# wtfashwin/fraud-detection

Measured on AMD Instinct MI355X. Metric: train_rows_per_sec (SMOTE k-NN + logistic fit, post-SMOTE rows/s, whole job); AUC; SHAP values/s, higher is better.
Workload: dtype bf16; 1 GPU; model=StandardScaler+SMOTE(k=5)+LogisticRegression(C=1,sgd), global_batch=8000000, seq_len=30, parallelism=dp1, rows_per_gpu=10000000, post_smote_rows_global=15972800, smote_scope=global

## Files before the change

fraud_detection_amd/csrc/kernels/knn.hip:

```cpp
#include <cmath>
#include <cstdlib>

#include "common.h"
#include "launchers.h"
#include "scaler_finalize.h"

namespace fdx {
namespace {

constexpr int kThreads = 256;
constexpr int kWaves = 4;
constexpr int kMaxK = 8;
constexpr float kNegBig = -3.0e38f;
constexpr int kQFlush = 4;
constexpr int kQCap = kQFlush - 1 + 16 + 1;

__device__ __forceinline__ bool better(float s, int i, float s2, int i2) {
  return s > s2 || (s == s2 && i < i2);
}

template <int K>
__device__ __forceinline__ void topk_insert(float (&bs)[K], int (&bi)[K], float s, int i) {
  if (!better(s, i, bs[K - 1], bi[K - 1])) return;
  bs[K - 1] = s;
  bi[K - 1] = i;
#pragma unroll
  for (int k = K - 1; k > 0; --k) {
    if (better(bs[k], bi[k], bs[k - 1], bi[k - 1])) {
      const float ts = bs[k]; bs[k] = bs[k - 1]; bs[k - 1] = ts;
      const int ti = bi[k]; bi[k] = bi[k - 1]; bi[k - 1] = ti;
    }
  }
}

__device__ __forceinline__ void split_row(const float (&x)[32], uint32_t (&h)[16], uint32_t (&l)[16]);
template <bool RAW>
__device__ __forceinline__ float4 prep_load(const float4* __restrict__ p, int k, const float* st, int d) {
#pragma clang fp contract(off)
  float4 v = p[k];
  if constexpr (RAW) {
    const int c = 4 * k;
    if (c < d) v.x = (v.x - st[c]) * st[32 + c];
    if (c + 1 < d) v.y = (v.y - st[c + 1]) * st[32 + c + 1];
    if (c + 2 < d) v.z = (v.z - st[c + 2]) * st[32 + c + 2];
    if (c + 3 < d) v.w = (v.w - st[c + 3]) * st[32 + c + 3];
  }
  return v;
}
template <bool RAW>
__device__ __forceinline__ void knn_prep_body(const float* __restrict__ X, int m, int m_pad, int role,
                                              float* __restrict__ out, float* __restrict__ outq,
                                              const double* __restrict__ aff, uint16_t* __restrict__ P,
                                              uint4* __restrict__ chl, uint4* __restrict__ qhl,
                                              float* __restrict__ tmax, const float* st, int d) {
#pragma clang fp contract(off)
  const int r = blockIdx.x * blockDim.x + threadIdx.x;
  if (chl != nullptr) {
    const bool ok = r < m_pad;
    float x[32];
    if (ok && r < m) {
      const float4* p = reinterpret_cast<const float4*>(X + (int64_t)r * kCols);
      float s = 0.0f;
#pragma unroll
      for (int k = 0; k < kCols / 4; ++k) {
        float4 v = prep_load<RAW>(p, k, st, d);
        if (k == kCols / 4 - 1) {
          s = fmaf(v.x, v.x, s); s = fmaf(v.y, v.y, s);
          v.z = 0.0f; v.w = 0.0f;
        } else {
          s = fmaf(v.x, v.x, s); s = fmaf(v.y, v.y, s); s = fmaf(v.z, v.z, s); s = fmaf(v.w, v.w, s);
        }
        x[4 * k] = v.x; x[4 * k + 1] = v.y; x[4 * k + 2] = v.z; x[4 * k + 3] = v.w;
      }
      x[30] = -0.5f * s;
    } else {
#pragma unroll
      for (int k = 0; k < 32; ++k) x[k] = 0.0f;
      x[30] = -3.0e38f;
    }
    uint32_t h[16], l[16];
    split_row(x, h, l);
    if (ok) {
      const int64_t tb = (int64_t)(r >> 5) * 256 + (r & 31);
#pragma unroll
      for (int v = 0; v < 8; ++v) {
        const int k = v & 3;
        const uint4 c = v < 4 ? make_uint4(h[4 * k], h[4 * k + 1], h[4 * k + 2], h[4 * k + 3])
                              : make_uint4(l[4 * k], l[4 * k + 1], l[4 * k + 2], l[4 * k + 3]);
        chl[tb + (v >> 1) * 64 + (v & 1) * 32] = c;
      }
    }
    float n2 = (ok && x[30] > -1.0e37f) ? -2.0f * x[30] : 0.0f;
#pragma unroll
    for (int o = 1; o < 32; o <<= 1) n2 = fmaxf(n2, __shfl_xor(n2, o, kWave));
    if (ok && (r & 31) == 0) tmax[r >> 5] = sqrtf(n2) * 1.0001f;
    x[30] = (ok && r < m) ? 1.0f : 0.0f;
    split_row(x, h, l);
    if (ok) {
#pragma unroll
      for (int k = 0; k < 4; ++k) {
        qhl[(int64_t)r * 8 + k] = make_uint4(h[4 * k], h[4 * k + 1], h[4 * k + 2], h[4 * k + 3]);
        qhl[(int64_t)r * 8 + 4 + k] = make_uint4(l[4 * k], l[4 * k + 1], l[4 * k + 2], l[4 * k + 3]);
      }
    }
  }
  if (r >= m_pad) return;
  float4* o = reinterpret_cast<float4*>(out + (int64_t)r * kCols);
  float4* oq = role == 2 ? reinterpret_cast<float4*>(outq + (int64_t)r * kCols) : nullptr;
  if (r >= m) {
#pragma unroll
    for (int k = 0; k < kCols / 4; ++k) {
      o[k] = make_float4(0.f, 0.f, 0.f, 0.f);
      if (oq) oq[k] = make_float4(0.f, 0.f, 0.f, 0.f);
    }
    if (role != 1) out[(int64_t)r * kCols + 30] = -3.0e38f;
    return;
  }
  const float4* p = reinterpret_cast<const float4*>(X + (int64_t)r * kCols);
  uint2* pp = P ? reinterpret_cast<uint2*>(P + (int64_t)r * kCols) : nullptr;
  float s = 0.0f;
#pragma unroll
  for (int k = 0; k < kCols / 4; ++k) {
    float4 v = prep_load<RAW>(p, k, st, d);
    if (pp) {
      float4 u = v;
      if constexpr (RAW) {
        const int c = 4 * k;
        u.x = u.x * st[64 + c] + st[96 + c];
        u.y = u.y * st[64 + c + 1] + st[96 + c + 1];
        if (c + 2 < kBiasCol) {
          u.z = u.z * st[64 + c + 2] + st[96 + c + 2];
          u.w = u.w * st[64 + c + 3] + st[96 + c + 3];
        }
      } else if (aff != nullptr) {
        const int c = 4 * k;
        u.x = u.x * (float)(1.0 / aff[32 + c]) + (float)aff[c];
        u.y = u.y * (float)(1.0 / aff[32 + c + 1]) + (float)aff[c + 1];
        if (c + 2 < kBiasCol) {
          u.z = u.z * (float)(1.0 / aff[32 + c + 2]) + (float)aff[c + 2];
          u.w = u.w * (float)(1.0 / aff[32 + c + 3]) + (float)aff[c + 3];
        }
      }
      pp[k] = make_uint2(pack_bf16x2(u.x, u.y), pack_bf16x2(u.z, u.w));
    }
    if (k == kCols / 4 - 1) {
      s = fmaf(v.x, v.x, s); s = fmaf(v.y, v.y, s);
      v.z = 0.0f; v.w = 0.0f;
    } else {
      s = fmaf(v.x, v.x, s); s = fmaf(v.y, v.y, s); s = fmaf(v.z, v.z, s); s = fmaf(v.w, v.w, s);
    }
    o[k] = v;
    if (oq) oq[k] = v;
  }
  out[(int64_t)r * kCols + 30] = role == 1 ? 1.0f : -0.5f * s;
  if (oq) outq[(int64_t)r * kCols + 30] = 1.0f;
}


__global__ void knn_prep_kernel(const float* __restrict__ X, int m, int m_pad, int role,
                                float* __restrict__ out, float* __restrict__ outq,
                                const double* __restrict__ aff, uint16_t* __restrict__ P,
                                uint4* __restrict__ chl = nullptr, uint4* __restrict__ qhl = nullptr,
                                float* __restrict__ tmax = nullptr) {
  knn_prep_body<false>(X, m, m_pad, role, out, outq, aff, P, chl, qhl, tmax, nullptr, 0);
}

__global__ __launch_bounds__(256) void knn_prep_raw_kernel(const float* __restrict__ X, int m, int m_pad,
                                                           float* __restrict__ out, float* __restrict__ outq,
                                                           uint16_t* __restrict__ P, uint4* __restrict__ chl,
                                                           uint4* __restrict__ qhl, float* __restrict__ tmax,
                                                           KnnRawStats st) {
  __shared__ float sst[4 * 32];
  if (threadIdx.x < 32) {
    const int c = threadIdx.x;
    float mu, inv;
    double ac, ai;
    if (st.nparts > 0) {
      const ScalerCol o = scaler_finalize_col(st.sums, st.n, st.pivot, st.d, st.colscale, st.nparts, c);
      mu = o.mean32; inv = o.inv32; ac = o.aff_c; ai = o.aff_inv;
      if (blockIdx.x == 0) {
        st.mean64[c] = o.mean; st.var64[c] = o.var; st.scale64[c] = o.scale;
        st.mean32[c] = mu; st.inv32[c] = inv;
        st.aff[c] = ac; st.aff[32 + c] = ai;
      }
    } else {
      mu = st.mean32[c]; inv = st.inv32[c]; ac = st.aff[c]; ai = st.aff[32 + c];
    }
    sst[c] = mu;
    sst[32 + c] = inv;
    sst[64 + c] = (float)(1.0 / ai);
    sst[96 + c] = (float)ac;
  }
  __syncthreads();
  knn_prep_body<true>(X, m, m_pad, 2, out, outq, nullptr, P, chl, qhl, tmax, sst, st.d);
}

template <int K, int QF = kQFlush>
__global__ __launch_bounds__(kWave) void knn_topk_kernel(const float* __restrict__ Q, int mq,
                                                         const float* __restrict__ C,
                                                         int mc_pad, int mc,
                                                         int64_t self_offset,
                                                         int* __restrict__ out_idx,
                                                         float* __restrict__ out_score) {
  const int lane = threadIdx.x;
  const int h = lane >> 5, j = lane & 31;
  const int q0 = blockIdx.x * 32;
  const int qg = q0 + j;
  const int64_t self_c = self_offset >= 0 ? self_offset + qg : -1;
  float bq[16];
  {
    const float4* p = reinterpret_cast<const float4*>(Q + (int64_t)qg * kCols + 16 * h);
#pragma unroll
    for (int k = 0; k < 4; ++k) {
      const float4 v = p[k];
      bq[4 * k] = v.x; bq[4 * k + 1] = v.y; bq[4 * k + 2] = v.z; bq[4 * k + 3] = v.w;
    }
  }
  float bs[K];
  int bi[K];
#pragma unroll
  for (int k = 0; k < K; ++k) { bs[k] = kNegBig; bi[k] = 0x7fffffff; }
  float thr = qg < mq ? kNegBig : __builtin_inff();

  constexpr int kCap = QF - 1 + 16 + 1;
  __shared__ int2 qent[kCap * kWave];
  int qn = 0;
  auto flush = [&]() {
    for (int e = 0; __any(e < qn); ++e) {
      if (e < qn) {
        const int2 v = qent[e * kWave + lane];
        const int ci = v.y;
        if (ci != self_c && ci < mc) topk_insert<K>(bs, bi, __int_as_float(v.x), ci);
      }
    }
    qn = 0;
    float ps[K];
#pragma unroll
    for (int k = 0; k < K; ++k) ps[k] = __shfl_xor(bs[k], 32, kWave);
    int ia = 0, ib = 0;
    float kth = kNegBig;
#pragma unroll
    for (int k = 0; k < K; ++k) {
      float a = kNegBig, b = kNegBig;
#pragma unroll
      for (int u = 0; u < K; ++u) { if (u == ia) a = bs[u]; if (u == ib) b = ps[u]; }
      const bool ta = a >= b;
      kth = ta ? a : b;
      ia += ta ? 1 : 0;
      ib += ta ? 0 : 1;
    }
    thr = qg < mq ? kth : __builtin_inff();
  };
  const int all_tiles = mc_pad / 32;
  const int t_lo = (int)(((int64_t)all_tiles * blockIdx.y) / gridDim.y);
  const int t_hi = (int)(((int64_t)all_tiles * (blockIdx.y + 1)) / gridDim.y);
  float4 cv[4];
  auto fetch = [&](int t, float4 (&a)[4]) {
    const float4* p = reinterpret_cast<const float4*>(C + (int64_t)(t * 32 + j) * kCols + 16 * h);
#pragma unroll
    for (int k = 0; k < 4; ++k) a[k] = p[k];
  };
  if (t_lo < t_hi) fetch(t_lo, cv);
  for (int t = t_lo; t < t_hi; ++t) {
    const int c0 = t * 32;
    float ac[16];
    f32x16_t acc = {};
#pragma unroll
    for (int k = 0; k < 4; ++k) {
      ac[4 * k] = cv[k].x; ac[4 * k + 1] = cv[k].y; ac[4 * k + 2] = cv[k].z; ac[4 * k + 3] = cv[k].w;
    }
    if (t + 1 < t_hi) fetch(t + 1, cv);
#pragma unroll
    for (int s = 0; s < 16; ++s) acc = __builtin_amdgcn_mfma_f32_32x32x2f32(ac[s], bq[s], acc, 0, 0, 0);
    float m4[4];
#pragma unroll
    for (int q = 0; q < 4; ++q) m4[q] = fmaxf(fmaxf(acc[4 * q], acc[4 * q + 1]), fmaxf(acc[4 * q + 2], acc[4 * q + 3]));
    const float mx = fmaxf(fmaxf(m4[0], m4[1]), fmaxf(m4[2], m4[3]));
    if (!__any(mx >= thr)) continue;
    const int cbase = c0 + 4 * h;
    int qe = qn * kWave + lane;
#pragma unroll
    for (int q = 0; q < 4; ++q) {
      if (!__any(m4[q] >= thr)) continue;
#pragma unroll
      for (int rr = 0; rr < 4; ++rr) {
        const int r = 4 * q + rr;
        const bool pass = acc[r] >= thr;
        if (__any(pass)) {
          if (pass) {
            qent[qe] = make_int2(__float_as_int(acc[r]), cbase + rr + 8 * q);
            qe += kWave;
          }
        }
      }
    }
    qn = (qe - lane) / kWave;
    if (__any(qn >= QF)) flush();
  }
  flush();
#pragma unroll
  for (int k = 0; k < K; ++k) {
    const float s2 = __shfl_xor(bs[k], 32, kWave);
    const int i2 = __shfl_xor(bi[k], 32, kWave);
    if (h == 0) topk_insert<K>(bs, bi, s2, i2);
  }
  if (h == 0 && qg < mq) {
    const int64_t o = ((int64_t)blockIdx.y * mq + qg) * K;
#pragma unroll
    for (int k = 0; k < K; ++k) {
      out_idx[o + k] = bi[k];
      if (out_score) out_score[o + k] = bs[k];
    }
  }
}

constexpr int kLW = 4;
constexpr int kCh = 2;
constexpr int kLdC = kCols + 4;

template <int K>
__global__ __launch_bounds__(kLW * kWave) void knn_topk_lds_kernel(const float* __restrict__ Q, int mq,
                                                                   const float* __restrict__ C, int mc_pad, int mc,
                                                                   int64_t self_offset, int* __restrict__ out_idx,
                                                                   float* __restrict__ out_score) {
  const int lane = lane_id(), wv = wave_id();
  const int h = lane >> 5, j = lane & 31;
  const int qg = (blockIdx.x * kLW + wv) * 32 + j;
  const int64_t self_c = self_offset >= 0 ? self_offset + qg : -1;
  __shared__ __attribute__((aligned(16))) float cbuf[2][kCh * 32 * kLdC];
  __shared__ int2 qall[kLW][kQCap * kWave];
  int2* qent = qall[wv];
  float bq[16];
  {
    const float4* p = reinterpret_cast<const float4*>(Q + (int64_t)qg * kCols + 16 * h);
#pragma unroll
    for (int k = 0; k < 4; ++k) {
      const float4 v = p[k];
      bq[4 * k] = v.x; bq[4 * k + 1] = v.y; bq[4 * k + 2] = v.z; bq[4 * k + 3] = v.w;
    }
  }
  float bs[K];
  int bi[K];
#pragma unroll
  for (int k = 0; k < K; ++k) { bs[k] = kNegBig; bi[k] = 0x7fffffff; }
  float thr = qg < mq ? kNegBig : __builtin_inff();
  int qn = 0;
  auto flush = [&]() {
    for (int e = 0; __any(e < qn); ++e) {
      if (e < qn) {
        const int2 v = qent[e * kWave + lane];
        const int ci = v.y;
        if (ci != self_c && ci < mc) topk_insert<K>(bs, bi, __int_as_float(v.x), ci);
      }
    }
    qn = 0;
    float ps[K];
#pragma unroll
    for (int k = 0; k < K; ++k) ps[k] = __shfl_xor(bs[k], 32, kWave);
    int ia = 0, ib = 0;
    float kth = kNegBig;
#pragma unroll
    for (int k = 0; k < K; ++k) {
      float a = kNegBig, b = kNegBig;
#pragma unroll
      for (int u = 0; u < K; ++u) { if (u == ia) a = bs[u]; if (u == ib) b = ps[u]; }
      const bool ta = a >= b;
      kth = ta ? a : b;
      ia += ta ? 1 : 0;
      ib += ta ? 0 : 1;
    }
    thr = qg < mq ? kth : __builtin_inff();
  };
  const int all_tiles = mc_pad / 32;
  const int t_lo = (int)(((int64_t)all_tiles * blockIdx.y) / gridDim.y);
  const int t_hi = (int)(((int64_t)all_tiles * (blockIdx.y + 1)) / gridDim.y);
  constexpr int kVec = kCh * 32 * 8 / (kLW * kWave);
  float4 st[kVec];
  auto load = [&](int c) {
    const int64_t r0 = (int64_t)(t_lo + kCh * c) * 32;
    const int64_t rmax = (int64_t)t_hi * 32;
#pragma unroll
    for (int i = 0; i < kVec; ++i) {
      const int e = threadIdx.x + i * kLW * kWave;
      const int64_t r = r0 + (e >> 3);
      st[i] = r < rmax ? reinterpret_cast<const float4*>(C + r * kCols)[e & 7] : make_float4(0.f, 0.f, 0.f, 0.f);
    }
  };
  auto store = [&](int b) {
#pragma unroll
    for (int i = 0; i < kVec; ++i) {
      const int e = threadIdx.x + i * kLW * kWave;
      *reinterpret_cast<float4*>(&cbuf[b][(e >> 3) * kLdC + 4 * (e & 7)]) = st[i];
    }
  };
  const int nch = (t_hi - t_lo + kCh - 1) / kCh;
  if (nch > 0) {
    load(0);
    store(0);
  }
  __syncthreads();
  for (int c = 0; c < nch; ++c) {
    if (c + 1 < nch) load(c + 1);
    const float* cb = cbuf[c & 1];
    const int ntile = min(kCh, t_hi - (t_lo + kCh * c));
    for (int tt = 0; tt < ntile; ++tt) {
      const int c0 = (t_lo + kCh * c + tt) * 32;
      const float* crow = cb + (tt * 32 + j) * kLdC + 16 * h;
      float ac[16];
#pragma unroll
      for (int k = 0; k < 4; ++k) {
        const float4 v = *reinterpret_cast<const float4*>(crow + 4 * k);
        ac[4 * k] = v.x; ac[4 * k + 1] = v.y; ac[4 * k + 2] = v.z; ac[4 * k + 3] = v.w;
      }
      f32x16_t acc = {};
#pragma unroll
      for (int s = 0; s < 16; ++s) acc = __builtin_amdgcn_mfma_f32_32x32x2f32(ac[s], bq[s], acc, 0, 0, 0);
      float mx = acc[0];
#pragma unroll
      for (int r = 1; r < 16; ++r) mx = fmaxf(mx, acc[r]);
      if (!__any(mx >= thr)) continue;
      const int cbase = c0 + 4 * h;
      int qe = qn * kWave + lane;
#pragma unroll
      for (int r = 0; r < 16; ++r) {
        const bool pass = acc[r] >= thr;
        if (__any(pass)) {
          if (pass) {
            qent[qe] = make_int2(__float_as_int(acc[r]), cbase + (r & 3) + 8 * (r >> 2));
            qe += kWave;
          }
        }
      }
      qn = (qe - lane) / kWave;
      if (__any(qn >= kQFlush)) flush();
    }
    if (c + 1 < nch) store((c + 1) & 1);
    __syncthreads();
  }
  flush();
#pragma unroll
  for (int k = 0; k < K; ++k) {
    const float s2 = __shfl_xor(bs[k], 32, kWave);
    const int i2 = __shfl_xor(bi[k], 32, kWave);
    if (h == 0) topk_insert<K>(bs, bi, s2, i2);
  }
  if (h == 0 && qg < mq) {
    const int64_t o = ((int64_t)blockIdx.y * mq + qg) * K;
#pragma unroll
    for (int k = 0; k < K; ++k) {
      out_idx[o + k] = bi[k];
      if (out_score) out_score[o + k] = bs[k];
    }
  }
}


__device__ __forceinline__ void split_row(const float (&x)[32], uint32_t (&h)[16], uint32_t (&l)[16]) {
#pragma unroll
  for (int k = 0; k < 16; ++k) {
    const float a = x[2 * k], b = x[2 * k + 1];
    const uint32_t ph = pack_bf16x2(a, b);
    h[k] = ph;
    l[k] = pack_bf16x2(a - bf16lo(ph), b - bf16hi(ph));
  }
}

__global__ __launch_bounds__(256) void knn_split_kernel(const float* __restrict__ Xp, int m_pad, int role,
                                                        uint4* __restrict__ hl, float* __restrict__ tmax) {
  const int r = blockIdx.x * 256 + threadIdx.x;
  const bool ok = r < m_pad;
  float x[32];
  const float4* p = reinterpret_cast<const float4*>(Xp + (int64_t)(ok ? r : 0) * kCols);
#pragma unroll
  for (int k = 0; k < 8; ++k) {
    const float4 v = p[k];
    x[4 * k] = v.x; x[4 * k + 1] = v.y; x[4 * k + 2] = v.z; x[4 * k + 3] = v.w;
  }
  uint32_t h[16], l[16];
  split_row(x, h, l);
  if (ok && role == 2) {
    const int64_t tb = (int64_t)(r >> 5) * 256 + (r & 31);
#pragma unroll
    for (int v = 0; v < 8; ++v) {
      const int k = v & 3;
      const uint4 c = v < 4 ? make_uint4(h[4 * k], h[4 * k + 1], h[4 * k + 2], h[4 * k + 3])
                            : make_uint4(l[4 * k], l[4 * k + 1], l[4 * k + 2], l[4 * k + 3]);
      hl[tb + (v >> 1) * 64 + (v & 1) * 32] = c;
    }
  } else if (ok) {
#pragma unroll
    for (int k = 0; k < 4; ++k) {
      hl[(int64_t)r * 8 + k] = make_uint4(h[4 * k], h[4 * k + 1], h[4 * k + 2], h[4 * k + 3]);
      hl[(int64_t)r * 8 + 4 + k] = make_uint4(l[4 * k], l[4 * k + 1], l[4 * k + 2], l[4 * k + 3]);
    }
  }
  if (role == 0 || role == 2) {
    float n2 = (ok && x[30] > -1.0e37f) ? -2.0f * x[30] : 0.0f;
// ... 568 lines not shown
  const int t_hi = (int)(((int64_t)all_tiles * (blockIdx.y + 1)) / gridDim.y);
  auto fetch = [&](int t, uint4 (&a)[4], float& tmv) {
    const uint4* p = Chl + (int64_t)t * 256 + lane;
    a[0] = p[0]; a[1] = p[64]; a[2] = p[128]; a[3] = p[192];
    tmv = tmax[t];
  };
  auto approx = [&](const uint4 (&c)[4]) -> f32x16_t {
    const bf16x8_t ch0 = __builtin_bit_cast(bf16x8_t, c[0]), ch1 = __builtin_bit_cast(bf16x8_t, c[1]);
    const bf16x8_t cl0 = __builtin_bit_cast(bf16x8_t, c[2]), cl1 = __builtin_bit_cast(bf16x8_t, c[3]);
    f32x16_t acc = {};
    acc = __builtin_amdgcn_mfma_f32_32x32x16_bf16(cl0, qh0, acc, 0, 0, 0);
    acc = __builtin_amdgcn_mfma_f32_32x32x16_bf16(cl1, qh1, acc, 0, 0, 0);
    acc = __builtin_amdgcn_mfma_f32_32x32x16_bf16(ch0, ql0, acc, 0, 0, 0);
    acc = __builtin_amdgcn_mfma_f32_32x32x16_bf16(ch1, ql1, acc, 0, 0, 0);
    acc = __builtin_amdgcn_mfma_f32_32x32x16_bf16(ch0, qh0, acc, 0, 0, 0);
    acc = __builtin_amdgcn_mfma_f32_32x32x16_bf16(ch1, qh1, acc, 0, 0, 0);
    return acc;
  };
  if (blockIdx.y > 0) {
    const int ns0 = (int)((int64_t)all_tiles / gridDim.y);
    const int nseed = ns0 < kSeedTiles ? ns0 : kSeedTiles;
    for (int t = 0; t < nseed; ++t) {
      uint4 c[4];
      float tm;
      fetch(t, c, tm);
      const f32x16_t acc = approx(c);
      (void)tm;
#pragma unroll
      for (int r = 0; r < 16; ++r) {
        const int ci = t * 32 + 4 * h + (r & 3) + 8 * (r >> 2);
        if (ci != self_c && ci < mc) topk_insert<kTopP>(bs, bi, acc[r], ci | kSeedFlag);
      }
    }
    const float kth = fmaxf(bs[kTopP - 1], __shfl_xor(bs[kTopP - 1], 32, kWave));
    thr = qg < mq ? kth : __builtin_inff();
  }
  constexpr int kBufs = 3;
  uint4 cb[kBufs][4];
  float tb[kBufs];
  const int tlast = t_hi > 0 ? t_hi - 1 : 0;
#pragma unroll
  for (int u = 0; u < kBufs; ++u) {
    fetch(t_lo + u < t_hi ? t_lo + u : tlast, cb[u], tb[u]);
    __builtin_amdgcn_sched_barrier(0);
  }
  for (int t0 = t_lo; t0 < t_hi; t0 += kBufs) {
#pragma unroll
    for (int u = 0; u < kBufs; ++u) {
      const int t = t0 + u;
      const f32x16_t acc = approx(cb[u]);
      const float tm = tb[u];
      fetch(t + kBufs < t_hi ? t + kBufs : tlast, cb[u], tb[u]);
      if (t >= t_hi) continue;
      const int c0 = t * 32;
      float mx = fmaxf(fmaxf(acc[0], acc[1]), acc[2]);
#pragma unroll
      for (int r = 3; r < 15; r += 2) mx = fmaxf(fmaxf(mx, acc[r]), acc[r + 1]);
      mx = fmaxf(mx, acc[15]);
      {
        const float mt = kMarginScale * fmaf(qn, tm, 0.5f * tm * tm);
        if (mx >= thr) mg_p = fmaxf(mg_p, mt);
        else ub_f = fmaxf(ub_f, mx + mt);
      }
      if (!__any(mx >= thr)) continue;
      uint32_t pm = 0;
#pragma unroll
      for (int r = 0; r < 16; ++r) pm |= (acc[r] >= thr ? 1u : 0u) << r;
      uint32_t wm = pm;
#pragma unroll
      for (int o = 1; o < kWave; o <<= 1) wm |= (uint32_t)__shfl_xor((int)wm, o, kWave);
      wm = __builtin_amdgcn_readfirstlane(wm);
      const int cbase = c0 + 4 * h;
      int qe = qn_ * kWave + lane;
      while (wm) {
        const int r = __builtin_ctz(wm);
        wm &= wm - 1;
        const int ci = cbase + (r & 3) + 8 * (r >> 2);
        if (((pm >> r) & 1u) && ci != self_c && ci < mc) {
          qent[qe] = make_int2(__float_as_int(acc[r]), ci);
          qe += kWave;
        }
      }
      qn_ = (qe - lane) / kWave;
      if (__any(qn_ >= QF)) flush();
    }
  }
  flush();
  ub_f = fmaxf(ub_f, __shfl_xor(ub_f, 32, kWave));
  mg_p = fmaxf(mg_p, __shfl_xor(mg_p, 32, kWave));
  float os[kTopP];
  int oi[kTopP];
#pragma unroll
  for (int k = 0; k < kTopP; ++k) {
    os[k] = __shfl_xor(bs[k], 32, kWave);
    oi[k] = __shfl_xor(bi[k], 32, kWave);
  }
  merge_sorted<kTopP>(bs, bi, os, oi);
  if (h == 0 && qg < mq) {
    const int64_t o = ((int64_t)blockIdx.y * mq + qg) * kTopP;
    int w = 0;
#pragma unroll
    for (int k = 0; k < kTopP; ++k) {
      if (bi[k] != 0x7fffffff && !(bi[k] & kSeedFlag)) {
        ws_s[o + w] = bs[k];
        ws_i[o + w] = bi[k];
        ++w;
      }
    }
    for (; w < kTopP; ++w) {
      ws_s[o + w] = kNegBig;
      ws_i[o + w] = 0x7fffffff;
    }
    ws_m[2 * ((int64_t)blockIdx.y * mq + qg)] = ub_f;
    ws_m[2 * ((int64_t)blockIdx.y * mq + qg) + 1] = mg_p;
  }
}

template <int K>
__global__ __launch_bounds__(256) void knn_b3top_final_kernel(const float* __restrict__ Q, const float* __restrict__ C,
                                                              int mq, int mc, int nsplit, int lps_log2,
                                                              int64_t self_offset, const float* __restrict__ ws_s,
                                                              const int* __restrict__ ws_i,
                                                              const float* __restrict__ ws_m,
                                                              int* __restrict__ out_idx, float* __restrict__ out_score,
                                                              int* __restrict__ fail) {
  const int lps = 1 << lps_log2;
  const int gl = blockIdx.x * 256 + threadIdx.x;
  const int q = gl >> lps_log2, sl = gl & (lps - 1);
  const bool live = q < mq;
  const int qq = live ? q : 0;
  const int64_t self_c = self_offset >= 0 ? self_offset + qq : -1;
  float as[kTopP];
  int ai[kTopP];
  float ub = kNegBig, mg = 0.0f;
#pragma unroll
  for (int k = 0; k < kTopP; ++k) { as[k] = kNegBig; ai[k] = 0x7fffffff; }
  if (live && sl < nsplit) {
    const int64_t o = ((int64_t)sl * mq + qq) * kTopP;
#pragma unroll
    for (int k = 0; k < kTopP; ++k) { as[k] = ws_s[o + k]; ai[k] = ws_i[o + k]; }
    ub = ws_m[2 * ((int64_t)sl * mq + qq)];
    mg = ws_m[2 * ((int64_t)sl * mq + qq) + 1];
  }
  for (int off = 1; off < lps; off <<= 1) {
    float os[kTopP];
    int oi[kTopP];
#pragma unroll
    for (int k = 0; k < kTopP; ++k) {
      os[k] = __shfl_xor(as[k], off, kWave);
      oi[k] = __shfl_xor(ai[k], off, kWave);
    }
    merge_sorted<kTopP>(as, ai, os, oi);
    mg = fmaxf(mg, __shfl_xor(mg, off, kWave));
    ub = fmaxf(ub, __shfl_xor(ub, off, kWave));
  }
  float qv[kCols];
  {
    const float4* p = reinterpret_cast<const float4*>(Q + (int64_t)qq * kCols);
#pragma unroll
    for (int k = 0; k < kCols / 4; ++k) {
      const float4 v = p[k];
      qv[4 * k] = v.x; qv[4 * k + 1] = v.y; qv[4 * k + 2] = v.z; qv[4 * k + 3] = v.w;
    }
  }
  auto exact = [&](int ci) -> float {
    const float4* c = reinterpret_cast<const float4*>(C + (int64_t)ci * kCols);
    float acc = 0.0f;
#pragma unroll
    for (int k = 0; k < kCols / 4; ++k) {
      const float4 v = c[k];
      acc = fmaf(qv[4 * k], v.x, acc);
      acc = fmaf(qv[4 * k + 1], v.y, acc);
      acc = fmaf(qv[4 * k + 2], v.z, acc);
      acc = fmaf(qv[4 * k + 3], v.w, acc);
    }
    return acc;
  };
  int my = 0x7fffffff;
#pragma unroll
  for (int u = 0; u < kTopP; ++u) if (u == sl) my = ai[u];
  const float ex = (my != 0x7fffffff && sl < kTopP) ? exact(my) : kNegBig;
  const int base = threadIdx.x & ~(lps - 1) & (kWave - 1);
  float bs[K];
  int bi[K];
#pragma unroll
  for (int k = 0; k < K; ++k) { bs[k] = kNegBig; bi[k] = 0x7fffffff; }
#pragma unroll
  for (int u = 0; u < kTopP; ++u) {
    const float e = __shfl(ex, base + u, kWave);
    if (ai[u] != 0x7fffffff) topk_insert<K>(bs, bi, e, ai[u]);
  }
  const float bound = fmaxf(ub, as[kTopP - 1] > kNegBig ? as[kTopP - 1] + mg : kNegBig);
  const bool ok = bs[K - 1] > bound;
  if (live && !ok && sl == 0) fail[1 + atomicAdd(fail, 1)] = q;
  if (live && sl == 0) {
#pragma unroll
    for (int k = 0; k < K; ++k) {
      out_idx[(int64_t)q * K + k] = bi[k];
      if (out_score) out_score[(int64_t)q * K + k] = bs[k];
    }
  }
}

template <int K>
__global__ __launch_bounds__(256) void knn_b3top_scan_kernel(const float* __restrict__ Q, const float* __restrict__ C,
                                                             int mc, int64_t self_offset, const int* __restrict__ fail,
                                                             int* __restrict__ out_idx, float* __restrict__ out_score) {
  const int nf = fail[0];
  __shared__ float ls[4][K];
  __shared__ int li[4][K];
  const int lane = lane_id(), wv = threadIdx.x >> 6;
  for (int f = blockIdx.x; f < nf; f += gridDim.x) {
    const int q = fail[1 + f];
    const int64_t self_c = self_offset >= 0 ? self_offset + q : -1;
    float qv[kCols];
    {
      const float4* p = reinterpret_cast<const float4*>(Q + (int64_t)q * kCols);
#pragma unroll
      for (int k = 0; k < kCols / 4; ++k) {
        const float4 v = p[k];
        qv[4 * k] = v.x; qv[4 * k + 1] = v.y; qv[4 * k + 2] = v.z; qv[4 * k + 3] = v.w;
      }
    }
    float bs[K];
    int bi[K];
#pragma unroll
    for (int k = 0; k < K; ++k) { bs[k] = kNegBig; bi[k] = 0x7fffffff; }
    for (int c0 = threadIdx.x; c0 < mc; c0 += 4 * 256) {
      float4 rv[4][kCols / 4];
#pragma unroll
      for (int u = 0; u < 4; ++u) {
        const int ci = c0 + u * 256;
        const float4* c = reinterpret_cast<const float4*>(C + (int64_t)(ci < mc ? ci : 0) * kCols);
#pragma unroll
        for (int k = 0; k < kCols / 4; ++k) rv[u][k] = c[k];
      }
#pragma unroll
      for (int u = 0; u < 4; ++u) {
        const int ci = c0 + u * 256;
        float acc = 0.0f;
#pragma unroll
        for (int k = 0; k < kCols / 4; ++k) {
          acc = fmaf(qv[4 * k], rv[u][k].x, acc);
          acc = fmaf(qv[4 * k + 1], rv[u][k].y, acc);
          acc = fmaf(qv[4 * k + 2], rv[u][k].z, acc);
          acc = fmaf(qv[4 * k + 3], rv[u][k].w, acc);
        }
        if (ci < mc && ci != self_c) topk_insert<K>(bs, bi, acc, ci);
      }
    }
    for (int off = 1; off < kWave; off <<= 1) {
      float os[K];
      int oi[K];
#pragma unroll
      for (int k = 0; k < K; ++k) {
        os[k] = __shfl_xor(bs[k], off, kWave);
        oi[k] = __shfl_xor(bi[k], off, kWave);
      }
      merge_sorted<K>(bs, bi, os, oi);
    }
    if (lane == 0) {
#pragma unroll
      for (int k = 0; k < K; ++k) { ls[wv][k] = bs[k]; li[wv][k] = bi[k]; }
    }
    __syncthreads();
    if (threadIdx.x == 0) {
      for (int w = 1; w < 4; ++w) {
        float os[K];
        int oi[K];
#pragma unroll
        for (int k = 0; k < K; ++k) { os[k] = ls[w][k]; oi[k] = li[w][k]; }
        merge_sorted<K>(bs, bi, os, oi);
      }
#pragma unroll
      for (int k = 0; k < K; ++k) {
        out_idx[(int64_t)q * K + k] = bi[k];
        if (out_score) out_score[(int64_t)q * K + k] = bs[k];
      }
    }
    __syncthreads();
  }
}

}

int merge_log2(int nsplit) {
  if (nsplit > kWave) throw std::runtime_error("knn merge: at most 64 candidate slices");
  int l = 0;
  while ((1 << l) < nsplit) ++l;
  return l;
}

unsigned merge_blocks(int mq, int nsplit) {
  return (unsigned)(((int64_t)mq << merge_log2(nsplit)) + 255) / 256;
}

void launch_knn_prep(const float* X, int m, int m_pad, int role, float* out, float* outq,
                     const double* aff, uint16_t* P, hipStream_t stream, void* chl, void* qhl, float* tmax) {
  if (role < 0 || role > 2 || (role == 2) != (outq != nullptr) || (role == 1 && P != nullptr))
    throw std::invalid_argument("knn_prep: role 2 needs outq (and only it); parents need a candidate role");
  if ((chl != nullptr || qhl != nullptr || tmax != nullptr) &&
      (role != 2 || chl == nullptr || qhl == nullptr || tmax == nullptr || m_pad % 32 != 0))
    throw std::invalid_argument("knn_prep: the fused split needs role 2, all three outputs and m_pad % 32 == 0");
  knn_prep_kernel<<<(m_pad + 255) / 256, 256, 0, stream>>>(X, m, m_pad, role, out, outq, aff, P,
                                                            static_cast<uint4*>(chl), static_cast<uint4*>(qhl), tmax);
  check_launch("knn_prep");
}

void launch_knn_prep_raw(const float* Xraw, int m, int m_pad, float* out, float* outq, uint16_t* P,
                         const KnnRawStats& st, hipStream_t stream, void* chl, void* qhl, float* tmax) {
  if (Xraw == nullptr || out == nullptr || outq == nullptr || m < 0 || m_pad < m)
    throw std::invalid_argument("knn_prep_raw: rows and both operand outputs");
  if ((chl != nullptr || qhl != nullptr || tmax != nullptr) &&
      (chl == nullptr || qhl == nullptr || tmax == nullptr || m_pad % 32 != 0))
    throw std::invalid_argument("knn_prep_raw: the fused split needs all three outputs and m_pad % 32 == 0");
  if (st.d < 1 || st.d > kCols - 2 || st.nparts < 0 || st.nparts > 128 || st.mean32 == nullptr ||
      st.inv32 == nullptr || st.aff == nullptr ||
      (st.nparts > 0 && (st.sums == nullptr || st.pivot == nullptr || st.mean64 == nullptr || st.var64 == nullptr ||
                         st.scale64 == nullptr)))
    throw std::invalid_argument("knn_prep_raw: bad statistics block");
  knn_prep_raw_kernel<<<(m_pad + 255) / 256, 256, 0, stream>>>(Xraw, m, m_pad, out, outq, P, static_cast<uint4*>(chl),
                                                                static_cast<uint4*>(qhl), tmax, st);
  check_launch("knn_prep_raw");
}

int knn_splits(int mq_pad, int mc_pad) {
  static const int cap = resident_cap(knn_topk_kernel<5>, kWave);
  const int qblocks = mq_pad / 32, tiles = mc_pad / 32;
  int max_s = tiles / 8;
  if (max_s > 32) max_s = 32;
  if (max_s < 1) max_s = 1;
  int best = 1;
  double best_eff = -1.0;
  for (int s = 1; s <= max_s; ++s) {
    const double blocks = (double)qblocks * s;
    const double rounds = std::ceil(blocks / cap);
    double eff = blocks / (rounds * cap);
    eff -= 0.004 * (s - 1);
    if (eff > best_eff + 1e-9) { best_eff = eff; best = s; }
  }
  return best;
}

int knn_lds_splits(int mq_pad, int mc_pad) {
  static const int cap = resident_cap(knn_topk_lds_kernel<5>, kLW * kWave);
  const int qblocks = mq_pad / (32 * kLW), tiles = mc_pad / 32;
  int max_s = tiles / (8 * kCh);
  if (max_s > 64) max_s = 64;
  if (max_s < 1) max_s = 1;
  int best = 1;
  double best_eff = -1.0;
  for (int s = 1; s <= max_s; ++s) {
    const double blocks = (double)qblocks * s;
    const double rounds = std::ceil(blocks / cap);
    double eff = blocks / (rounds * cap);
    eff -= 0.004 * (s - 1);
    if (eff > best_eff + 1e-9) { best_eff = eff; best = s; }
  }
  return best;
}

void launch_knn_topk_lds(const float* Q, int mq_pad, int mq, const float* C, int mc_pad, int mc,
                         int64_t self_offset, int k, int* out_idx, float* out_score, float* ws_score, int* ws_idx,
                         int nsplit, hipStream_t stream) {
  if (mq_pad % (32 * kLW) != 0 || mc_pad % 32 != 0)
    throw std::runtime_error("knn_topk_lds: query pad must be x128, candidate pad x32");
  if (nsplit < 1) nsplit = 1;
  if (nsplit > 1 && (ws_score == nullptr || ws_idx == nullptr))
    throw std::runtime_error("knn_topk_lds: split search needs the [nsplit][mq][k] workspaces");
  const dim3 grid(mq_pad / (32 * kLW), nsplit);
  int* oi = nsplit > 1 ? ws_idx : out_idx;
  float* os = nsplit > 1 ? ws_score : out_score;
#define FDX_KNNL(KK)                                                                                          \
  knn_topk_lds_kernel<KK><<<grid, kLW * kWave, 0, stream>>>(Q, mq, C, mc_pad, mc, self_offset, oi, os);       \
  if (nsplit > 1)                                                                                             \
    knn_merge_kernel<KK><<<merge_blocks(mq, nsplit), 256, 0, stream>>>(ws_score, ws_idx, nsplit, merge_log2(nsplit), mq, out_idx, out_score)
  switch (k) {
    case 1: FDX_KNNL(1); break;
    case 2: FDX_KNNL(2); break;
    case 3: FDX_KNNL(3); break;
    case 4: FDX_KNNL(4); break;
    case 5: FDX_KNNL(5); break;
    case 6: FDX_KNNL(6); break;
    case 7: FDX_KNNL(7); break;
    case 8: FDX_KNNL(8); break;
    default: throw std::runtime_error("knn_topk_lds: k must be in [1, 8]");
  }
#undef FDX_KNNL
  check_launch("knn_topk_lds");
}

void launch_knn_split(const float* Xp, int m_pad, int role, uint4* hl, float* tmax, hipStream_t stream) {
  knn_split_kernel<<<(m_pad + 255) / 256, 256, 0, stream>>>(Xp, m_pad, role, hl, tmax);
  check_launch("knn_split");
}

int knn3_splits(int mq_pad, int mc_pad) {
  static const int cap = resident_cap(knn_topk3_kernel<5>, kWave);
  const int qblocks = mq_pad / 32, tiles = mc_pad / 32;
  int max_s = tiles / 8;
  if (max_s > 32) max_s = 32;
  if (max_s < 1) max_s = 1;
  int best = 1;
  double best_eff = -1.0;
  for (int s = 1; s <= max_s; ++s) {
    const double blocks = (double)qblocks * s;
    const double rounds = std::ceil(blocks / cap);
    double eff = blocks / (rounds * cap);
    eff -= 0.004 * (s - 1);
    if (eff > best_eff + 1e-9) { best_eff = eff; best = s; }
  }
  return best;
}

void launch_knn_topk3(const float* Q, const void* Qhl, int mq_pad, int mq, const float* C, const void* Chl,
                      const float* tmax, int mc_pad, int mc, int64_t self_offset, int k, int* out_idx,
                      float* out_score, float* ws_score, int* ws_idx, int nsplit, hipStream_t stream) {
  if (mq_pad % 32 != 0 || mc_pad % 32 != 0) throw std::runtime_error("knn_topk3: pads must be x32");
  if (nsplit < 1) nsplit = 1;
  if (nsplit > 1 && (ws_score == nullptr || ws_idx == nullptr))
    throw std::runtime_error("knn_topk3: split search needs the [nsplit][mq][k] workspaces");
  const dim3 grid(mq_pad / 32, nsplit);
  int* oi = nsplit > 1 ? ws_idx : out_idx;
  float* os = nsplit > 1 ? ws_score : out_score;
  const uint4* qh = reinterpret_cast<const uint4*>(Qhl);
  const uint4* chl = reinterpret_cast<const uint4*>(Chl);
#define FDX_KNN3(KK)                                                                            \
  knn_topk3_kernel<KK><<<grid, kWave, 0, stream>>>(Q, qh, mq, C, chl, tmax, mc_pad, mc, self_offset, oi, os); \
  if (nsplit > 1)                                                                               \
    knn_merge_kernel<KK><<<merge_blocks(mq, nsplit), 256, 0, stream>>>(ws_score, ws_idx, nsplit, merge_log2(nsplit), mq, out_idx, out_score)
  switch (k) {
    case 1: FDX_KNN3(1); break;
    case 2: FDX_KNN3(2); break;
    case 3: FDX_KNN3(3); break;
    case 4: FDX_KNN3(4); break;
    case 5: FDX_KNN3(5); break;
    case 6: FDX_KNN3(6); break;
    case 7: FDX_KNN3(7); break;
    case 8: FDX_KNN3(8); break;
    default: throw std::runtime_error("knn_topk3: k must be in [1, 8]");
  }
#undef FDX_KNN3
  check_launch("knn_topk3");
}

int knn3r_list_cap() { return kListCap; }

int knn3r_splits(int mq_pad, int mc_pad) {
  (void)mq_pad;
  const int tiles = mc_pad / 32;
  int s = tiles / 16;
  if (s > 6) s = 6;
  if (s < 1) s = 1;
  return s;
}

void launch_knn_topk3r(const float* Q, const void* Qhl, int mq_pad, int mq, const float* C, const void* Chl,
                       const float* tmax, int mc_pad, int mc, int64_t self_offset, int k, int* out_idx,
                       float* out_score, int* lists, int* counts, int nsplit, hipStream_t stream) {
  int2* lists2 = reinterpret_cast<int2*>(lists);
  if (mq_pad % 32 != 0 || mc_pad % 32 != 0) throw std::runtime_error("knn_topk3r: pads must be x32");
  if (mq > mq_pad || mc > mc_pad || nsplit < 1 || lists == nullptr || counts == nullptr)
    throw std::runtime_error("knn_topk3r: bad shapes or missing list workspaces");
  const dim3 grid(mq_pad / 32, nsplit);
  const uint4* qh = reinterpret_cast<const uint4*>(Qhl);
  const uint4* chl = reinterpret_cast<const uint4*>(Chl);
  const unsigned rblocks = (unsigned)(((int64_t)mq * 8 + 255) / 256);
#define FDX_KNN3R(KK)                                                                                       \
  knn_collect_kernel<KK><<<grid, kWave, 0, stream>>>(Q, qh, chl, tmax, mq, mc_pad, mc, self_offset, lists2, counts); \
  knn_rerank_kernel<KK><<<rblocks, 256, 0, stream>>>(Q, C, mq, mc, mq_pad / 32, nsplit, self_offset, lists2, counts, \
                                                     out_idx, out_score)
  switch (k) {
    case 1: FDX_KNN3R(1); break;
    case 2: FDX_KNN3R(2); break;
    case 3: FDX_KNN3R(3); break;
    case 4: FDX_KNN3R(4); break;
    case 5: FDX_KNN3R(5); break;
    case 6: FDX_KNN3R(6); break;
    case 7: FDX_KNN3R(7); break;
    case 8: FDX_KNN3R(8); break;
    default: throw std::runtime_error("knn_topk3r: k must be in [1, 8]");
  }
#undef FDX_KNN3R
  check_launch("knn_topk3r");
}

int knn_b3top_splits(int mq_pad, int mc_pad) {
  static const int cap = resident_cap(knn_b3top_kernel<>, kWave);
  static const int forced = [] {
    const char* e = std::getenv("FDX_KNN_B3_SPLITS");
    return e != nullptr ? std::atoi(e) : 0;
  }();
  const int qblocks = mq_pad / 32, tiles = mc_pad / 32;
  int s = forced > 0 ? forced : cap / (qblocks > 0 ? qblocks : 1);
  if (s > 32) s = 32;
  if (s > tiles / 8) s = tiles / 8;
  if (s < 1) s = 1;
  return s;
}

void launch_knn_b3top(const float* Q, const void* Qhl, int mq_pad, int mq, const float* C, const void* Chl,
                      const float* tmax, int mc_pad, int mc, int64_t self_offset, int k, int* out_idx,
                      float* out_score, float* ws_s, int* ws_i, float* ws_m, int* fail, int nsplit,
                      hipStream_t stream) {
  if (mq_pad % 32 != 0 || mc_pad % 32 != 0) throw std::runtime_error("knn_b3top: pads must be x32");
  if (mq > mq_pad || mc > mc_pad || nsplit < 1 || nsplit > 32 || ws_s == nullptr || ws_i == nullptr || ws_m == nullptr)
    throw std::runtime_error("knn_b3top: bad shapes or missing [nsplit][mq][8] workspaces");
  if (fail == nullptr) throw std::runtime_error("knn_b3top: missing the [1 + mq] failed-query list");
  if (hipMemsetAsync(fail, 0, sizeof(int), stream) != hipSuccess) throw std::runtime_error("knn_b3top: memset");
  if (k < 1 || k > kTopP) throw std::runtime_error("knn_b3top: k must be in [1, 8]");
  const dim3 grid(mq_pad / 32, nsplit);
  knn_b3top_kernel<><<<grid, kWave, 0, stream>>>(Q, reinterpret_cast<const uint4*>(Qhl),
                                                  reinterpret_cast<const uint4*>(Chl), tmax, mq, mc_pad, mc,
                                                  self_offset, ws_s, ws_i, ws_m);
  int lg = merge_log2(nsplit);
  if (lg < 3) lg = 3;
  const unsigned fb = (unsigned)((((int64_t)mq << lg) + 255) / 256);
#define FDX_KNNB3(KK)                                                                                         \
  knn_b3top_final_kernel<KK><<<fb, 256, 0, stream>>>(Q, C, mq, mc, nsplit, lg, self_offset, ws_s, ws_i, ws_m, \
                                                     out_idx, out_score, fail);                                   \
  knn_b3top_scan_kernel<KK><<<256, 256, 0, stream>>>(Q, C, mc, self_offset, fail, out_idx, out_score)
  switch (k) {
    case 1: FDX_KNNB3(1); break;
    case 2: FDX_KNNB3(2); break;
    case 3: FDX_KNNB3(3); break;
    case 4: FDX_KNNB3(4); break;
    case 5: FDX_KNNB3(5); break;
    case 6: FDX_KNNB3(6); break;
    case 7: FDX_KNNB3(7); break;
    default: FDX_KNNB3(8); break;
  }
#undef FDX_KNNB3
  check_launch("knn_b3top");
}

void launch_knn_topk(const float* Q, int mq_pad, int mq, const float* C,
                     int mc_pad, int mc, int64_t self_offset, int k, int* out_idx,
                     float* out_score, float* ws_score, int* ws_idx, int nsplit, hipStream_t stream) {
  if (mq_pad % 32 != 0 || mc_pad % 32 != 0) throw std::runtime_error("knn_topk: pads must be x32");
  if (nsplit < 1) nsplit = 1;
  if (nsplit > 1 && (ws_score == nullptr || ws_idx == nullptr))
    throw std::runtime_error("knn_topk: split search needs the [nsplit][mq][k] workspaces");
  const dim3 grid(mq_pad / 32, nsplit);
  int* oi = nsplit > 1 ? ws_idx : out_idx;
  float* os = nsplit > 1 ? ws_score : out_score;
#define FDX_KNN(KK)                                                                             \
  knn_topk_kernel<KK><<<grid, kWave, 0, stream>>>(Q, mq, C, mc_pad, mc, self_offset, oi, os); \
  if (nsplit > 1)                                                                               \
    knn_merge_kernel<KK><<<merge_blocks(mq, nsplit), 256, 0, stream>>>(ws_score, ws_idx, nsplit, merge_log2(nsplit), mq, out_idx, out_score)
  switch (k) {
    case 1: FDX_KNN(1); break;
    case 2: FDX_KNN(2); break;
    case 3: FDX_KNN(3); break;
    case 4: FDX_KNN(4); break;
    case 5: FDX_KNN(5); break;
    case 6: FDX_KNN(6); break;
    case 7: FDX_KNN(7); break;
    case 8: FDX_KNN(8); break;
    default: throw std::runtime_error("knn_topk: k must be in [1, 8]");
  }
#undef FDX_KNN
  check_launch("knn_topk");
}

}
```

Measured before the change: 17.52 billion rows/s.

## Coalesce kNN prep loads and stores through a shared-memory row tile

The kNN prep kernels now run one 64-thread wave per 64-row block. Each block loads its rows cooperatively as contiguous float4s into an LDS tile, and the per-row results (operand rows, query hi/lo split, bf16 packed rows) are written back through the same tile so global stores are coalesced instead of strided per thread. The raw variant also starts the row fetch before the scaler finalize and stages the per-part column sums in LDS when there are at most 16 parts. In exchange it adds several barriers, reuses the LDS tile across phases, and launches smaller blocks, which may lower occupancy.

```diff
diff --git a/fraud_detection_amd/csrc/kernels/knn.hip b/fraud_detection_amd/csrc/kernels/knn.hip
--- a/fraud_detection_amd/csrc/kernels/knn.hip
+++ b/fraud_detection_amd/csrc/kernels/knn.hip
@@ -47,37 +47,105 @@
   }
   return v;
 }
+constexpr int kPrepRows = 64;
+constexpr int kPrepLd = kCols + 4;
+static_assert(kPrepRows % 32 == 0 && kPrepRows == kWave, "whole 32-row tiles (tmax's shuffles), one wave");
+
+__device__ __forceinline__ void prep_fetch(const float* __restrict__ X, int m, float4 (&ld)[8]) {
+  const int64_t base = (int64_t)blockIdx.x * kPrepRows;
+  const float4* src = reinterpret_cast<const float4*>(X) + base * 8;
+#pragma unroll
+  for (int i = 0; i < 8; ++i) {
+    const int e = threadIdx.x + kPrepRows * i;
+    ld[i] = base + (e >> 3) < m ? src[e] : make_float4(0.f, 0.f, 0.f, 0.f);
+  }
+}
+
 template <bool RAW>
-__device__ __forceinline__ void knn_prep_body(const float* __restrict__ X, int m, int m_pad, int role,
+__device__ __forceinline__ void knn_prep_body(const float4 (&ld)[8], float* tile, int m, int m_pad, int role,
                                               float* __restrict__ out, float* __restrict__ outq,
                                               const double* __restrict__ aff, uint16_t* __restrict__ P,
                                               uint4* __restrict__ chl, uint4* __restrict__ qhl,
                                               float* __restrict__ tmax, const float* st, int d) {
 #pragma clang fp contract(off)
-  const int r = blockIdx.x * blockDim.x + threadIdx.x;
+  const int tid = threadIdx.x;
+  const int64_t base = (int64_t)blockIdx.x * kPrepRows;
+  const int r = blockIdx.x * kPrepRows + tid;
+  const bool ok = r < m_pad, real = r < m;
+#pragma unroll
+  for (int i = 0; i < 8; ++i) {
+    const int e = tid + kPrepRows * i;
+    *reinterpret_cast<float4*>(&tile[(e >> 3) * kPrepLd + 4 * (e & 7)]) = ld[i];
+  }
+  __syncthreads();
+  float* mine = &tile[tid * kPrepLd];
+  float x[32];
+  uint2 pk[8];
+#pragma unroll
+  for (int k = 0; k < 8; ++k) pk[k] = make_uint2(0u, 0u);
+  if (real) {
+    const float4* p = reinterpret_cast<const float4*>(mine);
+    float s = 0.0f;
+#pragma unroll
+    for (int k = 0; k < kCols / 4; ++k) {
+      float4 v = prep_load<RAW>(p, k, st, d);
+      if (P != nullptr) {
+        float4 u = v;
+        if constexpr (RAW) {
+          const int c = 4 * k;
+          u.x = u.x * st[64 + c] + st[96 + c];
+          u.y = u.y * st[64 + c + 1] + st[96 + c + 1];
+          if (c + 2 < kBiasCol) {
+            u.z = u.z * st[64 + c + 2] + st[96 + c + 2];
+            u.w = u.w * st[64 + c + 3] + st[96 + c + 3];
+          }
+        } else if (aff != nullptr) {
+          const int c = 4 * k;
+          u.x = u.x * (float)(1.0 / aff[32 + c]) + (float)aff[c];
+          u.y = u.y * (float)(1.0 / aff[32 + c + 1]) + (float)aff[c + 1];
+          if (c + 2 < kBiasCol) {
+            u.z = u.z * (float)(1.0 / aff[32 + c + 2]) + (float)aff[c + 2];
+            u.w = u.w * (float)(1.0 / aff[32 + c + 3]) + (float)aff[c + 3];
+          }
+        }
+        pk[k] = make_uint2(pack_bf16x2(u.x, u.y), pack_bf16x2(u.z, u.w));
+      }
+      if (k == kCols / 4 - 1) {
+        s = fmaf(v.x, v.x, s); s = fmaf(v.y, v.y, s);
+        v.z = 0.0f; v.w = 0.0f;
+      } else {
+        s = fmaf(v.x, v.x, s); s = fmaf(v.y, v.y, s); s = fmaf(v.z, v.z, s); s = fmaf(v.w, v.w, s);
+      }
+      x[4 * k] = v.x; x[4 * k + 1] = v.y; x[4 * k + 2] = v.z; x[4 * k + 3] = v.w;
+    }
+    x[30] = role == 1 ? 1.0f : -0.5f * s;
+  } else {
+#pragma unroll
+    for (int k = 0; k < 32; ++k) x[k] = 0.0f;
+    x[30] = role == 1 ? 0.0f : -3.0e38f;
+  }
+#pragma unroll
+  for (int k = 0; k < 8; ++k)
+    *reinterpret_cast<float4*>(mine + 4 * k) = make_float4(x[4 * k], x[4 * k + 1], x[4 * k + 2], x[4 * k + 3]);
+  __syncthreads();
+  {
+    float4* o4 = reinterpret_cast<float4*>(out) + base * 8;
+    float4* q4 = outq != nullptr ? reinterpret_cast<float4*>(outq) + base * 8 : nullptr;
+#pragma unroll
+    for (int i = 0; i < 8; ++i) {
+      const int e = tid + kPrepRows * i;
+      const int64_t row = base + (e >> 3);
+      if (row < m_pad) {
+        float4 v = *reinterpret_cast<const float4*>(&tile[(e >> 3) * kPrepLd + 4 * (e & 7)]);
+        o4[e] = v;
+        if (q4 != nullptr) {
+          if ((e & 7) == 7) v.z = row < m ? 1.0f : 0.0f;
+          q4[e] = v;
+        }
+      }
+    }
+  }
   if (chl != nullptr) {
-    const bool ok = r < m_pad;
-    float x[32];
-    if (ok && r < m) {
-      const float4* p = reinterpret_cast<const float4*>(X + (int64_t)r * kCols);
-      float s = 0.0f;
-#pragma unroll
-      for (int k = 0; k < kCols / 4; ++k) {
-        float4 v = prep_load<RAW>(p, k, st, d);
-        if (k == kCols / 4 - 1) {
-          s = fmaf(v.x, v.x, s); s = fmaf(v.y, v.y, s);
-          v.z = 0.0f; v.w = 0.0f;
-        } else {
-          s = fmaf(v.x, v.x, s); s = fmaf(v.y, v.y, s); s = fmaf(v.z, v.z, s); s = fmaf(v.w, v.w, s);
-        }
-        x[4 * k] = v.x; x[4 * k + 1] = v.y; x[4 * k + 2] = v.z; x[4 * k + 3] = v.w;
-      }
-      x[30] = -0.5f * s;
-    } else {
-#pragma unroll
-      for (int k = 0; k < 32; ++k) x[k] = 0.0f;
-      x[30] = -3.0e38f;
-    }
     uint32_t h[16], l[16];
     split_row(x, h, l);
     if (ok) {
@@ -94,89 +162,81 @@
 #pragma unroll
     for (int o = 1; o < 32; o <<= 1) n2 = fmaxf(n2, __shfl_xor(n2, o, kWave));
     if (ok && (r & 31) == 0) tmax[r >> 5] = sqrtf(n2) * 1.0001f;
-    x[30] = (ok && r < m) ? 1.0f : 0.0f;
+    x[30] = real ? 1.0f : 0.0f;
     split_row(x, h, l);
-    if (ok) {
-#pragma unroll
-      for (int k = 0; k < 4; ++k) {
-        qhl[(int64_t)r * 8 + k] = make_uint4(h[4 * k], h[4 * k + 1], h[4 * k + 2], h[4 * k + 3]);
-        qhl[(int64_t)r * 8 + 4 + k] = make_uint4(l[4 * k], l[4 * k + 1], l[4 * k + 2], l[4 * k + 3]);
-      }
-    }
-  }
-  if (r >= m_pad) return;
-  float4* o = reinterpret_cast<float4*>(out + (int64_t)r * kCols);
-  float4* oq = role == 2 ? reinterpret_cast<float4*>(outq + (int64_t)r * kCols) : nullptr;
-  if (r >= m) {
-#pragma unroll
-    for (int k = 0; k < kCols / 4; ++k) {
-      o[k] = make_float4(0.f, 0.f, 0.f, 0.f);
-      if (oq) oq[k] = make_float4(0.f, 0.f, 0.f, 0.f);
-    }
-    if (role != 1) out[(int64_t)r * kCols + 30] = -3.0e38f;
-    return;
-  }
-  const float4* p = reinterpret_cast<const float4*>(X + (int64_t)r * kCols);
-  uint2* pp = P ? reinterpret_cast<uint2*>(P + (int64_t)r * kCols) : nullptr;
-  float s = 0.0f;
-#pragma unroll
-  for (int k = 0; k < kCols / 4; ++k) {
-    float4 v = prep_load<RAW>(p, k, st, d);
-    if (pp) {
-      float4 u = v;
-      if constexpr (RAW) {
-        const int c = 4 * k;
-        u.x = u.x * st[64 + c] + st[96 + c];
-        u.y = u.y * st[64 + c + 1] + st[96 + c + 1];
-        if (c + 2 < kBiasCol) {
-          u.z = u.z * st[64 + c + 2] + st[96 + c + 2];
-          u.w = u.w * st[64 + c + 3] + st[96 + c + 3];
-        }
-      } else if (aff != nullptr) {
-        const int c = 4 * k;
-        u.x = u.x * (float)(1.0 / aff[32 + c]) + (float)aff[c];
-        u.y = u.y * (float)(1.0 / aff[32 + c + 1]) + (float)aff[c + 1];
-        if (c + 2 < kBiasCol) {
-          u.z = u.z * (float)(1.0 / aff[32 + c + 2]) + (float)aff[c + 2];
-          u.w = u.w * (float)(1.0 / aff[32 + c + 3]) + (float)aff[c + 3];
-        }
-      }
-      pp[k] = make_uint2(pack_bf16x2(u.x, u.y), pack_bf16x2(u.z, u.w));
-    }
-    if (k == kCols / 4 - 1) {
-      s = fmaf(v.x, v.x, s); s = fmaf(v.y, v.y, s);
-      v.z = 0.0f; v.w = 0.0f;
-    } else {
-      s = fmaf(v.x, v.x, s); s = fmaf(v.y, v.y, s); s = fmaf(v.z, v.z, s); s = fmaf(v.w, v.w, s);
-    }
-    o[k] = v;
-    if (oq) oq[k] = v;
-  }
-  out[(int64_t)r * kCols + 30] = role == 1 ? 1.0f : -0.5f * s;
-  if (oq) outq[(int64_t)r * kCols + 30] = 1.0f;
-}
-
-
-__global__ void knn_prep_kernel(const float* __restrict__ X, int m, int m_pad, int role,
-                                float* __restrict__ out, float* __restrict__ outq,
-                                const double* __restrict__ aff, uint16_t* __restrict__ P,
-                                uint4* __restrict__ chl = nullptr, uint4* __restrict__ qhl = nullptr,
-                                float* __restrict__ tmax = nullptr) {
-  knn_prep_body<false>(X, m, m_pad, role, out, outq, aff, P, chl, qhl, tmax, nullptr, 0);
-}
-
-__global__ __launch_bounds__(256) void knn_prep_raw_kernel(const float* __restrict__ X, int m, int m_pad,
-                                                           float* __restrict__ out, float* __restrict__ outq,
-                                                           uint16_t* __restrict__ P, uint4* __restrict__ chl,
-                                                           uint4* __restrict__ qhl, float* __restrict__ tmax,
-                                                           KnnRawStats st) {
+    __syncthreads();
+    uint4* mine4 = reinterpret_cast<uint4*>(mine);
+#pragma unroll
+    for (int k = 0; k < 4; ++k) {
+      mine4[k] = make_uint4(h[4 * k], h[4 * k + 1], h[4 * k + 2], h[4 * k + 3]);
+      mine4[4 + k] = make_uint4(l[4 * k], l[4 * k + 1], l[4 * k + 2], l[4 * k + 3]);
+    }
+    __syncthreads();
+    uint4* g = qhl + base * 8;
+#pragma unroll
+    for (int i = 0; i < 8; ++i) {
+      const int e = tid + kPrepRows * i;
+      if (base + (e >> 3) < m_pad) g[e] = *reinterpret_cast<const uint4*>(&tile[(e >> 3) * kPrepLd + 4 * (e & 7)]);
+    }
+  }
+  if (P != nullptr) {
+    __syncthreads();
+    uint2* mine2 = reinterpret_cast<uint2*>(mine);
+#pragma unroll
+    for (int k = 0; k < 8; ++k) mine2[k] = pk[k];
+    __syncthreads();
+    uint4* g = reinterpret_cast<uint4*>(P) + base * 4;
+#pragma unroll
+    for (int i = 0; i < 4; ++i) {
+      const int e = tid + kPrepRows * i;
+      if (base + (e >> 2) < m) g[e] = *reinterpret_cast<const uint4*>(&tile[(e >> 2) * kPrepLd + 4 * (e & 3)]);
+    }
+  }
+}
+
+__global__ __launch_bounds__(kPrepRows) void knn_prep_kernel(const float* __restrict__ X, int m, int m_pad, int role,
+                                                             float* __restrict__ out, float* __restrict__ outq,
+                                                             const double* __restrict__ aff, uint16_t* __restrict__ P,
+                                                             uint4* __restrict__ chl = nullptr,
+                                                             uint4* __restrict__ qhl = nullptr,
+                                                             float* __restrict__ tmax = nullptr) {
+  __shared__ __attribute__((aligned(16))) float tile[kPrepRows * kPrepLd];
+  float4 ld[8];
+  prep_fetch(X, m, ld);
+  knn_prep_body<false>(ld, tile, m, m_pad, role, out, outq, aff, P, chl, qhl, tmax, nullptr, 0);
+}
+
+__global__ __launch_bounds__(kPrepRows) void knn_prep_raw_kernel(const float* __restrict__ X, int m, int m_pad,
+                                                                 float* __restrict__ out, float* __restrict__ outq,
+                                                                 uint16_t* __restrict__ P, uint4* __restrict__ chl,
+                                                                 uint4* __restrict__ qhl, float* __restrict__ tmax,
+                                                                 KnnRawStats st) {
+  __shared__ __attribute__((aligned(16))) float tile[kPrepRows * kPrepLd];
   __shared__ float sst[4 * 32];
+  float4 ld[8];
+  prep_fetch(X, m, ld);
+  constexpr int kStageParts = 16;
+  const bool staged = st.nparts > 0 && st.nparts <= kStageParts;
+  double* sp = reinterpret_cast<double*>(tile);
+  if (staged) {
+#pragma unroll
+    for (int p0 = 0; p0 < kStageParts; p0 += 8) {
+      double v[8];
+#pragma unroll
+      for (int i = 0; i < 8; ++i) v[i] = p0 + i < st.nparts ? st.sums[(p0 + i) * 64 + threadIdx.x] : 0.0;
+#pragma unroll
+      for (int i = 0; i < 8; ++i)
+        if (p0 + i < st.nparts) sp[(p0 + i) * 64 + threadIdx.x] = v[i];
+    }
+    __syncthreads();
+  }
   if (threadIdx.x < 32) {
     const int c = threadIdx.x;
     float mu, inv;
     double ac, ai;
     if (st.nparts > 0) {
-      const ScalerCol o = scaler_finalize_col(st.sums, st.n, st.pivot, st.d, st.colscale, st.nparts, c);
+      const ScalerCol o = staged ? scaler_finalize_col(sp, st.n, st.pivot, st.d, st.colscale, st.nparts, c)
+                                 : scaler_finalize_col(st.sums, st.n, st.pivot, st.d, st.colscale, st.nparts, c);
       mu = o.mean32; inv = o.inv32; ac = o.aff_c; ai = o.aff_inv;
       if (blockIdx.x == 0) {
         st.mean64[c] = o.mean; st.var64[c] = o.var; st.scale64[c] = o.scale;
@@ -192,7 +252,7 @@
     sst[96 + c] = (float)ac;
   }
   __syncthreads();
-  knn_prep_body<true>(X, m, m_pad, 2, out, outq, nullptr, P, chl, qhl, tmax, sst, st.d);
+  knn_prep_body<true>(ld, tile, m, m_pad, 2, out, outq, nullptr, P, chl, qhl, tmax, sst, st.d);
 }
 
 template <int K, int QF = kQFlush>
@@ -1367,8 +1427,8 @@
   if ((chl != nullptr || qhl != nullptr || tmax != nullptr) &&
       (role != 2 || chl == nullptr || qhl == nullptr || tmax == nullptr || m_pad % 32 != 0))
     throw std::invalid_argument("knn_prep: the fused split needs role 2, all three outputs and m_pad % 32 == 0");
-  knn_prep_kernel<<<(m_pad + 255) / 256, 256, 0, stream>>>(X, m, m_pad, role, out, outq, aff, P,
-                                                            static_cast<uint4*>(chl), static_cast<uint4*>(qhl), tmax);
+  knn_prep_kernel<<<(m_pad + kPrepRows - 1) / kPrepRows, kPrepRows, 0, stream>>>(
+      X, m, m_pad, role, out, outq, aff, P, static_cast<uint4*>(chl), static_cast<uint4*>(qhl), tmax);
   check_launch("knn_prep");
 }
 
@@ -1384,8 +1444,8 @@
       (st.nparts > 0 && (st.sums == nullptr || st.pivot == nullptr || st.mean64 == nullptr || st.var64 == nullptr ||
                          st.scale64 == nullptr)))
     throw std::invalid_argument("knn_prep_raw: bad statistics block");
-  knn_prep_raw_kernel<<<(m_pad + 255) / 256, 256, 0, stream>>>(Xraw, m, m_pad, out, outq, P, static_cast<uint4*>(chl),
-                                                                static_cast<uint4*>(qhl), tmax, st);
+  knn_prep_raw_kernel<<<(m_pad + kPrepRows - 1) / kPrepRows, kPrepRows, 0, stream>>>(
+      Xraw, m, m_pad, out, outq, P, static_cast<uint4*>(chl), static_cast<uint4*>(qhl), tmax, st);
   check_launch("knn_prep_raw");
 }
 
```

Result: no change. 17.60 billion rows/s, median of 6 (+0.5%).
